# neeek2303/EMOPortraits

Measured on AMD Instinct MI355X. Metric: reenactment frames/sec @512x512, 1-src->N-driver, higher is better.
Workload: dtype f32

## Files before the change

### emoportraits_amd/build.py

```python
import concurrent.futures
import hashlib
import os
import subprocess
import sys

HERE = os.path.dirname(os.path.abspath(__file__))
CSRC = os.path.join(HERE, "csrc")
LIBDIR = os.path.join(HERE, "lib")
LIB = os.path.join(LIBDIR, "libemoportraits_hip.so")
OBJDIR = os.path.join(LIBDIR, "obj")
HIPCC = os.environ.get("HIPCC", "/opt/rocm/bin/hipcc")
ARCH = "gfx950"
FLAGS = ["--offload-arch=" + ARCH, "-O3", "-std=c++17", "-fPIC", "-ffp-contract=off", "-Wall",
         "-Wno-unused-function", "-Wno-unused-variable", "-mllvm", "-pragma-unroll-threshold=100000"]


EXTRA_FLAGS = {"gs3d_tile_pad_zeros.hip": ["-fno-slp-vectorize"], "gs3d_tile_pad_border.hip": ["-fno-slp-vectorize"],
               "gs3d_tile_pad_reflection.hip": ["-fno-slp-vectorize"],
               "conv_inst_bf16x3_3x3.hip": ["-fno-slp-vectorize"], "conv_inst_f16x2_3x3.hip": ["-fno-slp-vectorize"],
               "conv_inst_f16x2_ct2.hip": ["-fno-slp-vectorize"], "conv_inst_f16x2_p1.hip": ["-fno-slp-vectorize"],
               "conv_inst_f16x2_w8.hip": ["-fno-slp-vectorize"], "conv_inst_f16x2_up2.hip": ["-fno-slp-vectorize"]}


def sources():
    return sorted(os.path.join(CSRC, f) for f in os.listdir(CSRC) if f.endswith(".hip"))


def _digest(paths):
    h = hashlib.sha256()
    for p in sorted(paths):
        with open(p, "rb") as f:
            h.update(p.encode())
            h.update(f.read())
    h.update(" ".join(FLAGS).encode())
    for p in sorted(paths):
        h.update(" ".join(EXTRA_FLAGS.get(os.path.basename(p), [])).encode())
    return h.hexdigest()


def _compile(src):
    hdrs = [os.path.join(CSRC, f) for f in os.listdir(CSRC) if f.endswith(".h")]
    hdrs.append(os.path.join(HERE, "..", "include", "emo_hip.h"))
    dig = _digest([src] + hdrs)
    obj = os.path.join(OBJDIR, os.path.basename(src) + ".o")
    stamp = obj + ".sha"
    if os.path.exists(obj) and os.path.exists(stamp) and open(stamp).read() == dig:
        return obj, False
    extra = EXTRA_FLAGS.get(os.path.basename(src), [])
    cmd = [HIPCC] + FLAGS + extra + ["-c", src, "-o", obj]
    r = subprocess.run(cmd, capture_output=True, text=True)
    if r.returncode != 0:
        raise RuntimeError("hipcc failed for %s:\n%s\n%s" % (src, r.stdout, r.stderr))
    if r.stderr.strip():
        sys.stderr.write(r.stderr)
    with open(stamp, "w") as f:
        f.write(dig)
    return obj, True


def build_variant(name, defines):
    global FLAGS, OBJDIR, LIB
    saved = (FLAGS, OBJDIR, LIB)
    try:
        FLAGS = FLAGS + ["-D" + d for d in defines]
        OBJDIR = os.path.join(LIBDIR, "obj_" + name)
        LIB = os.path.join(LIBDIR, f"libemoportraits_hip_{name}.so")
        return build(force=False, verbose=True)
    finally:
        FLAGS, OBJDIR, LIB = saved


def build(force=False, verbose=True):
    os.makedirs(OBJDIR, exist_ok=True)
    srcs = sources()
    if force:
        for f in os.listdir(OBJDIR):
            os.remove(os.path.join(OBJDIR, f))
    with concurrent.futures.ThreadPoolExecutor(max_workers=min(8, len(srcs))) as ex:
        results = list(ex.map(_compile, srcs))
    objs = [o for o, _ in results]
    rebuilt = any(r for _, r in results)
    if rebuilt or not os.path.exists(LIB):
        cmd = [HIPCC, "--offload-arch=" + ARCH, "-shared", "-fPIC", "-o", LIB] + objs
        r = subprocess.run(cmd, capture_output=True, text=True)
        if r.returncode != 0:
            raise RuntimeError("link failed:\n%s\n%s" % (r.stdout, r.stderr))
        if verbose:
            print("built", LIB)
    elif verbose:
        print("up to date:", LIB)
    return LIB


if __name__ == "__main__":
    if "--variant" in sys.argv:
        i = sys.argv.index("--variant")
        build_variant(sys.argv[i + 1], sys.argv[i + 2:])
    else:
        build(force="--force" in sys.argv)
```

### emoportraits_amd/csrc/conv_api.hip

```cpp
#include "conv_dispatch.h"

conv_launch_fn conv_lookup_3x3_A(int, int);
conv_launch_fn conv_lookup_3x3_B(int, int);
conv_launch_fn conv_lookup_3x3_C(int, int);
conv_launch_fn conv_lookup_3x3_D(int, int);
conv_launch_fn conv_lookup_3x3_E(int, int);
conv_launch_fn conv_lookup_3x3_F(int, int);
conv_launch_fn conv_lookup_1x1_A(int, int);
conv_launch_fn conv_lookup_1x1_B(int, int);
conv_launch_fn conv_lookup_1x1_C(int, int);
conv_launch_fn conv_lookup_1x7_A(int, int);
conv_launch_fn conv_lookup_1x7_B(int, int);
conv_launch_fn conv_lookup_f16_3x3_D(int, int);
conv_launch_fn conv_lookup_f16_1x1_D(int, int);
conv_launch_fn conv_lookup_f16_3x3_G(int, int);
conv_launch_fn conv_lookup_bf16x3_3x3(int, int);
conv_launch_fn conv_lookup_f16x2_3x3(int, int);
conv_launch_fn conv_lookup_f16x2_1x1(int, int);
conv_launch_fn conv_lookup_f16x2_3x3_bm32(int, int);
conv_launch_fn conv_lookup_f16w8_3x3(int, int);
int conv_f16x2_up2_launch(ConvArgs, hipStream_t);

enum { PREC_F32 = 0, PREC_F16 = 1, PREC_S = 2, PREC_S2 = 3, PREC_H1 = 4, PREC_S2U = 5 };

static int shape_of_width(int Wl) {
  if (Wl >= 128 && Wl % 128 == 0) return SHAPE_W128;
  if (Wl == 64) return SHAPE_W64;
  if (Wl == 32) return SHAPE_W32;
  if (Wl == 16) return SHAPE_W16;
  if (Wl == 8) return SHAPE_W8;
  return -1;
}

static int kc_of(int KH, int KW, int cfg, int prec = PREC_F32) {
  if (prec == PREC_H1) return (cfg == CFG_D && KH == 3 && KW == 3) ? 32 : 0;
  if (prec == PREC_S2U) return (cfg == CFG_D && KH == 3 && KW == 3) ? 16 : 0;
  if (prec == PREC_S2 && cfg == CFG_D && KH == 1 && KW == 1) return 32;
  if (prec == PREC_S2 && cfg == CFG_F && KH == 3 && KW == 3) return 16;
  if (prec == PREC_S || prec == PREC_S2) return (cfg == CFG_D && KH == 3 && KW == 3) ? 16 : 0;
  if (prec == PREC_F16) {
    if (cfg == CFG_G) return (KH == 3 && KW == 3) ? EMO_CONV_KC_F16_3X3 : 0;
    if (cfg != CFG_D) return 0;
    return (KH == 3 && KW == 3) ? EMO_CONV_KC_F16_3X3 : (KH == 1 && KW == 1) ? EMO_CONV_KC_F16_1X1 : 0;
  }
  if (cfg == CFG_G) return 0;
  if (KH == 3 && KW == 3) return cfg == CFG_A ? EMO_CONV_KC_3X3_A : EMO_CONV_KC_3X3;
  if (cfg == CFG_D || cfg == CFG_E || cfg == CFG_F) return 0;
  if (KH == 1 && KW == 1) return EMO_CONV_KC_1X1;
  if (KH == 1 && KW == 7) return EMO_CONV_KC_1X7;
  return 0;
}

extern "C" int emo_conv_pack_info(int KH, int KW, int cfg, int* BM, int* KC) {
  if (!BM || !KC) return EMO_ERR_BAD_ARG;
  if (cfg == CFG_A) *BM = 128; else if (cfg == CFG_B || cfg == CFG_D || cfg == CFG_E) *BM = 64; else if (cfg == CFG_C || cfg == CFG_F) *BM = 32; else return EMO_ERR_BAD_ARG;
  *KC = kc_of(KH, KW, cfg);
  return *KC ? EMO_OK : EMO_ERR_UNSUPPORTED;
}

extern "C" int emo_conv_tile_positions(int cfg) {
  if (cfg == CFG_A || cfg == CFG_B || cfg == CFG_C) return 128;
  if (cfg == CFG_D || cfg == CFG_F || cfg == CFG_G) return 256;
  if (cfg == CFG_E) return 512;
  return EMO_ERR_BAD_ARG;
}

__global__ __launch_bounds__(256) void conv_splitk_epilogue_kernel(const float* __restrict__ partial,
                                                                   const float* __restrict__ bias, const float* res,
                                                                   float* out, long total, int ksplit, int Cout, int Dl,
                                                                   int Hl, int Wl, int act, int res_ups, const int* run_if) {
  if (run_if != nullptr && *run_if == 0) return;
  const long ovol = (long)Dl * Hl * Wl;
  for (long i = (long)blockIdx.x * 256 + threadIdx.x; i < total; i += (long)gridDim.x * 256) {
    float v = partial[i];
    for (int k = 1; k < ksplit; ++k) v += partial[(long)k * total + i];
    const long nc = i / ovol;
    if (bias) v += bias[nc % Cout];
    if (res) {
      if (res_ups) {
        const long sp = i - nc * ovol;
        const int x = (int)(sp % Wl);
        const long r = sp / Wl;
        const int y = (int)(r % Hl), z = (int)(r / Hl);
        const int Wr = Wl >> 1, Hr = Hl >> 1;
        v += res[nc * ((long)Dl * Hr * Wr) + ((long)z * Hr + (y >> 1)) * Wr + (x >> 1)];
      } else {
        v += res[i];
      }
    }
    out[i] = emo_act(v, act);
  }
}


extern "C" int emo_conv_pack_info_f16(int KH, int KW, int cfg, int* BM, int* KC) {
  if (!BM || !KC) return EMO_ERR_BAD_ARG;
  if (cfg == CFG_D) *BM = 64; else if (cfg == CFG_G) *BM = 128; else return EMO_ERR_UNSUPPORTED;
  *KC = kc_of(KH, KW, cfg, PREC_F16);
  return *KC ? EMO_OK : EMO_ERR_UNSUPPORTED;
}

extern "C" int emo_conv_pack_info_bf16x3(int KH, int KW, int cfg, int* BM, int* KC) {
  if (!BM || !KC) return EMO_ERR_BAD_ARG;
  if (cfg != CFG_D) return EMO_ERR_UNSUPPORTED;
  *BM = 64;
  *KC = kc_of(KH, KW, cfg, PREC_S);
  return *KC ? EMO_OK : EMO_ERR_UNSUPPORTED;
}

extern "C" int emo_conv_igemm_ksplit(int N, int Cin, int Cout, int D, int H, int W, int KD, int KH, int KW, int ups,
                                     int cfg) {
  const int kc = kc_of(KH, KW, cfg);
  if (!kc || N <= 0 || Cin <= 0 || Cout <= 0 || D <= 0 || H <= 0 || W <= 0 || cfg < 0 || cfg >= N_CFGS) return EMO_ERR_BAD_ARG;
  const int bm = (cfg == CFG_A || cfg == CFG_G) ? 128 : (cfg == CFG_B || cfg == CFG_D || cfg == CFG_E) ? 64 : 32;
  const int bp = (cfg == CFG_D || cfg == CFG_F || cfg == CFG_G) ? 256 : cfg == CFG_E ? 512 : 128;
  const long pos = (long)N * D * (ups ? 4 : 1) * H * W;
  const long blocks = ((pos + bp - 1) / bp) * ((Cout + bm - 1) / bm);
  const int nstages = ((Cin + kc - 1) / kc) * KD;
  long want = blocks >= 512 ? 1 : (512 + blocks - 1) / blocks;
  if (want > nstages / 8) want = nstages / 8;
  if (want > 16) want = 16;
  return want < 1 ? 1 : (int)want;
}

static int conv_igemm_dispatch(int prec, const float* x, const void* wpk, const float* bias, const float* scale,
                               const float* shift, const float* res, float* out, int N, int Cin, int Cout, int D, int H,
                               int W, int KD, int KH, int KW, int ups, int relu_in, int act, int res_ups, int cfg,
                               int ksplit, float* workspace, float* gn_stats, void* stream, float in_scale = 1.0f,
                               float w_scale = 1.0f, int* sat_flag = nullptr, const int* run_if = nullptr, int cot0 = 0,
                               int cot_end = 0) {
  if (!x || !wpk || !out) return EMO_ERR_BAD_ARG;
  if (gn_stats && ksplit > 1) return EMO_ERR_UNSUPPORTED;
  if ((long)D * H * W >= (1L << 30)) return EMO_ERR_UNSUPPORTED;
  if (ksplit < 1 || (ksplit > 1 && !workspace)) return EMO_ERR_BAD_ARG;
  if (N <= 0 || Cin <= 0 || Cout <= 0 || D <= 0 || H <= 0 || W <= 0) return EMO_ERR_BAD_ARG;
  if ((scale == nullptr) != (shift == nullptr)) return EMO_ERR_BAD_ARG;
  if (KD != 1 && KD != 3 && KD != 7) return EMO_ERR_UNSUPPORTED;
  if (KD == 3 && !(KH == 3 && KW == 3)) return EMO_ERR_UNSUPPORTED;
  if ((KD == 7) != (KH == 1 && KW == 7)) return EMO_ERR_UNSUPPORTED;
  if (cfg < 0 || cfg >= N_CFGS) return EMO_ERR_BAD_ARG;
  if (!emo_aligned16(wpk)) return EMO_ERR_ALIGN;
  if (ups && D != 1) return EMO_ERR_UNSUPPORTED;
  if ((long)Cin * D * H * W >= (1L << 31)) return EMO_ERR_UNSUPPORTED;
  ConvArgs a;
  a.x = x; a.wpk = reinterpret_cast<const float*>(wpk); a.bias = bias; a.scale = scale; a.shift = shift; a.res = res; a.out = out;
  a.N = N; a.Cin = Cin; a.Cout = Cout; a.D = D; a.H = H; a.W = W;
  a.Dl = D; a.Hl = ups ? 2 * H : H; a.Wl = ups ? 2 * W : W;
  a.KD = KD; a.relu_in = relu_in; a.act = act; a.res_ups = res_ups;
  a.gn_stats = gn_stats;
  a.n_cchunks = 0; a.tiles_x = a.tiles_y = a.tiles_z = 0; a.n_cotiles = 0; a.n_work = 0; a.cot0 = cot0; a.cot_end = cot_end;
  if ((cot0 != 0 && !(prec == PREC_F16 && cfg == CFG_D && ksplit == 1)) || (cot_end != 0 && prec != PREC_H1)) return EMO_ERR_BAD_ARG;
  a.in_scale = in_scale; a.out_scale = 1.0f / (in_scale * w_scale);
  a.sat_flag = sat_flag; a.run_if = run_if;
  const int shape = shape_of_width(a.Wl);
  if (shape < 0) return EMO_ERR_UNSUPPORTED;
  conv_launch_fn fn = nullptr;
  if (prec == PREC_H1) {
    if (!(KH == 3 && KW == 3 && (KD == 1 || KD == 3)) || cfg != CFG_D || Cin % 8 || ksplit != 1 || run_if != nullptr) return EMO_ERR_UNSUPPORTED;
    if (!(in_scale > 0.0f && w_scale > 0.0f)) return EMO_ERR_BAD_ARG;
    fn = conv_lookup_f16w8_3x3(a.Wl, ups);
  } else if (prec == PREC_S2U) {
    if (!(KH == 3 && KW == 3 && KD == 1) || !ups || cfg != CFG_D || ksplit != 1 || run_if != nullptr) return EMO_ERR_UNSUPPORTED;
    if (!(in_scale > 0.0f && w_scale > 0.0f)) return EMO_ERR_BAD_ARG;
    fn = &conv_f16x2_up2_launch;
  } else if (prec == PREC_S2 && KH == 1 && KW == 1) {
    if (KD != 1 || cfg != CFG_D || Cin % 8 || ksplit != 1 || run_if != nullptr) return EMO_ERR_UNSUPPORTED;
    if (!(in_scale > 0.0f && w_scale > 0.0f)) return EMO_ERR_BAD_ARG;
    fn = conv_lookup_f16x2_1x1(a.Wl, ups);
  } else if (prec == PREC_S2 && cfg == CFG_F) {
    if (!(KH == 3 && KW == 3 && (KD == 1 || KD == 3)) || Cin % 8) return EMO_ERR_UNSUPPORTED;
    if (!(in_scale > 0.0f && w_scale > 0.0f)) return EMO_ERR_BAD_ARG;
    fn = conv_lookup_f16x2_3x3_bm32(a.Wl, ups);
  } else if (prec == PREC_S || prec == PREC_S2) {
    if (!(KH == 3 && KW == 3 && (KD == 1 || KD == 3)) || cfg != CFG_D || Cin % 8) return EMO_ERR_UNSUPPORTED;
    if (prec == PREC_S2 && !(in_scale > 0.0f && w_scale > 0.0f)) return EMO_ERR_BAD_ARG;
    fn = prec == PREC_S ? conv_lookup_bf16x3_3x3(a.Wl, ups) : conv_lookup_f16x2_3x3(a.Wl, ups);
  } else if (prec == PREC_F16) {
    if (KD != 1 && !(KD == 3 && KH == 3)) return EMO_ERR_UNSUPPORTED;
    if ((cfg != CFG_D && cfg != CFG_G) || Cin % 8) return EMO_ERR_UNSUPPORTED;
    if (cfg == CFG_G) fn = (KH == 3 && KW == 3) ? conv_lookup_f16_3x3_G(shape, ups) : nullptr;
    else if (KH == 3 && KW == 3) fn = conv_lookup_f16_3x3_D(shape, ups);
    else if (KH == 1 && KW == 1) fn = conv_lookup_f16_1x1_D(shape, ups);
    else return EMO_ERR_UNSUPPORTED;
  } else if (cfg == CFG_G) {
    return EMO_ERR_UNSUPPORTED;
  } else if (cfg == CFG_D || cfg == CFG_E || cfg == CFG_F) {
    if (!(KH == 3 && KW == 3 && (KD == 1 || (KD == 3 && cfg != CFG_E)))) return EMO_ERR_UNSUPPORTED;
    fn = cfg == CFG_D ? conv_lookup_3x3_D(shape, ups) : cfg == CFG_E ? conv_lookup_3x3_E(shape, ups) : conv_lookup_3x3_F(shape, ups);
  } else if (KH == 3 && KW == 3) {
    fn = cfg == CFG_A ? conv_lookup_3x3_A(shape, ups) : cfg == CFG_B ? conv_lookup_3x3_B(shape, ups) : conv_lookup_3x3_C(shape, ups);
  } else if (KH == 1 && KW == 1) {
    fn = cfg == CFG_A ? conv_lookup_1x1_A(shape, ups) : cfg == CFG_B ? conv_lookup_1x1_B(shape, ups) : conv_lookup_1x1_C(shape, ups);
  } else if (KH == 1 && KW == 7) {
    fn = cfg == CFG_A ? conv_lookup_1x7_A(shape, ups) : cfg == CFG_B ? conv_lookup_1x7_B(shape, ups) : nullptr;
  } else {
    return EMO_ERR_UNSUPPORTED;
  }
  if (!fn) return EMO_ERR_UNSUPPORTED;
  const int kc = kc_of(KH, KW, cfg, prec);
  if (!kc) return EMO_ERR_UNSUPPORTED;
  const int nstages = ((Cin + kc - 1) / kc) * KD;
  if (ksplit > nstages) ksplit = nstages;
  a.stages_per_split = (nstages + ksplit - 1) / ksplit;
  a.ksplit = (nstages + a.stages_per_split - 1) / a.stages_per_split;
  a.partial = a.ksplit > 1 ? workspace : nullptr;
  const int rc = fn(a, (hipStream_t)stream);
  if (rc != EMO_OK || a.ksplit == 1) return rc;
  const long total = (long)N * Cout * a.Dl * a.Hl * a.Wl;
  long blocks = (total + 255) / 256;
  if (blocks > 262144) blocks = 262144;
  hipLaunchKernelGGL(conv_splitk_epilogue_kernel, dim3((unsigned)blocks), dim3(256), 0, (hipStream_t)stream, workspace, bias,
                     res, out, total, a.ksplit, Cout, a.Dl, a.Hl, a.Wl, act, res_ups, run_if);
  return emo_launch_status();
}

extern "C" int emo_conv_igemm_f32(const float* x, const float* wpk, const float* bias, const float* scale,
                                  const float* shift, const float* res, float* out, int N, int Cin, int Cout, int D,
                                  int H, int W, int KD, int KH, int KW, int ups, int relu_in, int act, int res_ups,
                                  int cfg, int ksplit, float* workspace, float* gn_stats, void* stream) {
  return conv_igemm_dispatch(PREC_F32, x, wpk, bias, scale, shift, res, out, N, Cin, Cout, D, H, W, KD, KH, KW, ups,
                             relu_in, act, res_ups, cfg, ksplit, workspace, gn_stats, stream);
}

extern "C" int emo_conv_igemm_f32_guarded(const float* x, const float* wpk, const float* bias, const float* scale,
                                          const float* shift, const float* res, float* out, int N, int Cin, int Cout, int D,
                                          int H, int W, int KD, int KH, int KW, int ups, int relu_in, int act, int res_ups,
                                          int cfg, int ksplit, float* workspace, float* gn_stats, void* stream,
                                          const int* run_if) {
  return conv_igemm_dispatch(PREC_F32, x, wpk, bias, scale, shift, res, out, N, Cin, Cout, D, H, W, KD, KH, KW, ups,
                             relu_in, act, res_ups, cfg, ksplit, workspace, gn_stats, stream, 1.0f, 1.0f, nullptr, run_if);
}

extern "C" int emo_conv_igemm_bf16x3(const float* x, const void* wpk3, const float* bias, const float* scale,
                                     const float* shift, const float* res, float* out, int N, int Cin, int Cout, int D,
                                     int H, int W, int KD, int KH, int KW, int ups, int relu_in, int act, int res_ups,
                                     int cfg, int ksplit, float* workspace, float* gn_stats, void* stream,
                                     const int* run_if) {
  return conv_igemm_dispatch(PREC_S, x, wpk3, bias, scale, shift, res, out, N, Cin, Cout, D, H, W, KD, KH, KW, ups,
                             relu_in, act, res_ups, cfg, ksplit, workspace, gn_stats, stream, 1.0f, 1.0f, nullptr, run_if);
}

extern "C" int emo_conv_igemm_f16x2(const float* x, const void* wpk2, const float* bias, const float* scale,
                                    const float* shift, const float* res, float* out, int N, int Cin, int Cout, int D,
                                    int H, int W, int KD, int KH, int KW, int ups, int relu_in, int act, int res_ups,
                                    int cfg, int ksplit, float* workspace, float* gn_stats, void* stream, float in_scale,
                                    float w_scale, int* overflow_flag) {
  if (cfg == EMO_CONV_CFG_F16X2_UP2)
    return conv_igemm_dispatch(PREC_S2U, x, wpk2, bias, scale, shift, res, out, N, Cin, Cout, D, H, W, KD, KH, KW, ups,
                               relu_in, act, res_ups, CFG_D, ksplit, workspace, gn_stats, stream, in_scale, w_scale,
                               overflow_flag, nullptr);
  return conv_igemm_dispatch(PREC_S2, x, wpk2, bias, scale, shift, res, out, N, Cin, Cout, D, H, W, KD, KH, KW, ups,
                             relu_in, act, res_ups, cfg, ksplit, workspace, gn_stats, stream, in_scale, w_scale,
                             overflow_flag, nullptr);
}

extern "C" int emo_conv_igemm_f16acc32(const float* x, const void* wpk16, const float* bias, const float* scale,
                                       const float* shift, const float* res, float* out, int N, int Cin, int Cout, int D,
                                       int H, int W, int KD, int KH, int KW, int ups, int relu_in, int act, int res_ups,
                                       int cfg, int ksplit, float* workspace, float* gn_stats, void* stream) {
  return conv_igemm_dispatch(PREC_F16, x, wpk16, bias, scale, shift, res, out, N, Cin, Cout, D, H, W, KD, KH, KW, ups,
                             relu_in, act, res_ups, cfg, ksplit, workspace, gn_stats, stream);
}

extern "C" int emo_conv_igemm_f16w8_rest(const float* x, const void* wpk1, const void* wpk16, const float* bias,
                                         const float* scale, const float* shift, const float* res, float* out, int N, int Cin,
                                         int Cout, int D, int H, int W, int KD, int KH, int KW, int ups, int relu_in, int act,
                                         int res_ups, int cfg, int ksplit, float* workspace, float* gn_stats, void* stream,
                                         float w_scale) {
  const int cot = (Cout + 63) / 64;
  if (!wpk16 || Cout % 64 || cot < 3 || !(cot & 1)) return EMO_ERR_UNSUPPORTED;
  const int Wl = ups ? 2 * W : W, Hl = ups ? 2 * H : H;
  if (!((Wl % 128 == 0 && Hl % 2 == 0) || (Wl == 64 && Hl % 4 == 0))) return EMO_ERR_UNSUPPORTED;
  int rc = conv_igemm_dispatch(PREC_H1, x, wpk1, bias, scale, shift, res, out, N, Cin, Cout, D, H, W, KD, KH, KW, ups, relu_in,
                               act, res_ups, cfg, ksplit, workspace, gn_stats, stream, 1.0f, w_scale, nullptr, nullptr, 0, cot - 1);
  if (rc != EMO_OK) return rc;
  return conv_igemm_dispatch(PREC_F16, x, wpk16, bias, scale, shift, res, out, N, Cin, Cout, D, H, W, KD, KH, KW, ups, relu_in,
                             act, res_ups, cfg, ksplit, workspace, gn_stats, stream, 1.0f, 1.0f, nullptr, nullptr, cot - 1, 0);
}

extern "C" int emo_conv_igemm_f16w8(const float* x, const void* wpk1, const float* bias, const float* scale,
                                    const float* shift, const float* res, float* out, int N, int Cin, int Cout, int D,
                                    int H, int W, int KD, int KH, int KW, int ups, int relu_in, int act, int res_ups,
                                    int cfg, int ksplit, float* workspace, float* gn_stats, void* stream, float w_scale) {
  return conv_igemm_dispatch(PREC_H1, x, wpk1, bias, scale, shift, res, out, N, Cin, Cout, D, H, W, KD, KH, KW, ups,
                             relu_in, act, res_ups, cfg, ksplit, workspace, gn_stats, stream, 1.0f, w_scale, nullptr, nullptr);
}
```

### emoportraits_amd/csrc/conv_igemm.h

```cpp
#pragma once
#include "common.h"

#include <mutex>
#include <set>
#include <utility>

typedef float floatx16 __attribute__((ext_vector_type(16)));
typedef float floatx4 __attribute__((ext_vector_type(4)));

#ifndef EMO_CONV_MAX_WAVES
#define EMO_CONV_MAX_WAVES 5
#endif

struct ConvArgs {
  const float* x;
  const float* wpk;
  const float* bias;
  const float* scale;
  const float* shift;
  const float* res;
  float* out;
  int N, Cin, Cout;
  int D, H, W;
  int Dl, Hl, Wl;
  int KD;
  int relu_in;
  int act;
  int res_ups;
  int n_cchunks;
  int tiles_x, tiles_y, tiles_z;
  int n_cotiles;
  int cot0;
  int cot_end;
  float in_scale, out_scale;
  int n_work;
  int ksplit;
  int stages_per_split;
  float* partial;
  float* gn_stats;
  int* sat_flag;
  const int* run_if;
};

template <int KH, int KW, int KC, int TZ, int TR, int TW, int TM, int TP, int WGM, int WGP, bool UPS>
struct ConvCfg {
  static constexpr int BM = WGM * TM * 32;
  static constexpr int BP = WGP * TP * 32;
  static constexpr int TAPS = KH * KW;
  static constexpr int KLOC = KC * TAPS;
  static constexpr int PR = TR + KH - 1;
  static constexpr int PW = TW + KW - 1;
  static constexpr int CHS = TZ * PR * PW;
  static constexpr int PATCH = KC * CHS;
  static constexpr int ASZ = KLOC * BM;
  static constexpr int BUF = ASZ + ((PATCH + 3) & ~3);
  static constexpr int SW = 4;
  static constexpr int THREADS = 256;
  static constexpr int WPC = KC >= SW ? 1 : SW / KC;
  static constexpr int CPW = KC >= SW ? KC / SW : 1;
  static constexpr int EPC = (CHS + 64 * WPC - 1) / (64 * WPC);
  static constexpr int NPE = CPW * EPC;
  static constexpr int NSTEPS = (KC / 2) * TAPS;
  static_assert(WGM * WGP == 4, "4 waves per block");
  static_assert(TZ * TR * TW == BP, "position tile must equal BP");
  static_assert(KC % 2 == 0 && (KC % SW == 0 || SW % KC == 0), "whole channels per wave, or whole waves per channel");
  static_assert(ASZ % 4 == 0, "weight tile must be float4-copyable");
  static_assert(TM * TP <= 8, "accumulator budget");
  static_assert(2 * BUF >= 2 * WGP * BM, "the GroupNorm tile statistics are exchanged through the stage buffers");
  static constexpr int LDS_BYTES = (2 * BUF + 256) * 4;
  static constexpr int BY_LDS = (160 * 1024) / LDS_BYTES;
  static constexpr int CAP = TM * TP >= 8 ? 2
                             : TM * TP >= 4 ? (EMO_CONV_MAX_WAVES < 4 ? EMO_CONV_MAX_WAVES : 4)
                                            : EMO_CONV_MAX_WAVES;
  static constexpr int OCC = BY_LDS < 2 ? 2 : (BY_LDS > CAP ? CAP : BY_LDS);
};

__device__ __forceinline__ float emo_act(float v, int act) {
  if (act == EMO_ACT_RELU) return fmaxf(v, 0.0f);
  if (act == EMO_ACT_TANH) return tanhf(v);
  if (act == EMO_ACT_SIGMOID) return 1.0f / (1.0f + expf(-v));
  return v;
}

#ifndef EMO_SGPR_HAZARD_NOP
#define EMO_SGPR_HAZARD_NOP "s_nop 4\n\t"
#endif


__device__ __forceinline__ float emo_gload_pinned(const float* sbase, unsigned voff) {
  float v;
  asm volatile(EMO_SGPR_HAZARD_NOP "global_load_dword %0, %1, %2" : "=v"(v) : "v"(voff), "s"(sbase) : "memory");
  return v;
}
__device__ __forceinline__ floatx4 emo_gload4_pinned(const float* sbase, unsigned voff) {
  floatx4 v;
  asm volatile(EMO_SGPR_HAZARD_NOP "global_load_dwordx4 %0, %1, %2" : "=v"(v) : "v"(voff), "s"(sbase) : "memory");
  return v;
}
__device__ __forceinline__ void emo_touch4(floatx4& v) { asm volatile("" : "+v"(v)); }
__device__ __forceinline__ void emo_wait_vmem0() { asm volatile("s_waitcnt vmcnt(0)" ::: "memory"); }
__device__ __forceinline__ void emo_touch(float& v) { asm volatile("" : "+v"(v)); }

#define acc_at(i_, j_) ((j_) < TPH ? acc_lo[i_][(j_) < TPH ? (j_) : 0] : acc_hi[i_][(j_) >= TPH ? (j_) - TPH : 0])

#ifndef EMO_CONV_NT_STORE
#define EMO_CONV_NT_STORE 0
#endif
__device__ __forceinline__ void emo_store4(float* p, const floatx4& v, bool aligned) {
  if (aligned) {
    if (EMO_CONV_NT_STORE) __builtin_nontemporal_store(v, reinterpret_cast<floatx4*>(p));
    else *reinterpret_cast<floatx4*>(p) = v;
  } else {
    p[0] = v[0]; p[1] = v[1]; p[2] = v[2]; p[3] = v[3];
  }
}

template <int TZ, int TR, int TW, int TM, int TP, int WGP, int BM>
__device__ __forceinline__ void conv_epilogue(const ConvArgs& a, floatx16 (&acc_lo)[TM][TP > 2 ? TP / 2 : TP],
                                              floatx16 (&acc_hi)[TM][TP > 2 ? TP / 2 : TP], float* smem, int n, int cotile,
                                              int ptile, int ks, int x0, int y0, int z0, int m0, int p0, int wp, int half,
                                              int l32, int tid) {
  constexpr int TPH = TP > 2 ? TP / 2 : TP;
  static_assert(TW % 4 == 0, "4 consecutive positions of a register quad lie in one tile row");
  const long plane = (long)a.Hl * a.Wl;
  const long ovol = (long)a.Dl * plane;
  const bool to_partial = a.partial != nullptr;
  const bool has_bias = a.bias != nullptr && !to_partial;
  const bool has_res = a.res != nullptr && !to_partial;
  const bool out_al = ((reinterpret_cast<unsigned long long>(to_partial ? a.partial : a.out) & 15ull) == 0);
  const bool res_al = has_res && ((reinterpret_cast<unsigned long long>(a.res) & 15ull) == 0);
#pragma unroll
  for (int i = 0; i < TM; ++i) {
    const int co = cotile * BM + m0 + i * 32 + l32;
    const bool co_ok = co < a.Cout;
    const int cs = co_ok ? co : a.Cout - 1;
    const float bv = has_bias ? a.bias[cs] : 0.0f;
#pragma unroll
    for (int j = 0; j < TP; ++j) {
      long sp[4];
      floatx4 rv[4];
#pragma unroll
      for (int q = 0; q < 4; ++q) {
        const int p4 = p0 + j * 32 + 8 * q + 4 * half;
        const int col = p4 % TW;
        const int row = (p4 / TW) % TR;
        const int pz = p4 / (TW * TR);
        const int z = z0 + pz, y = y0 + row, x = x0 + col;
        sp[q] = (long)z * plane + (long)y * a.Wl + x;
        rv[q] = floatx4{0.0f, 0.0f, 0.0f, 0.0f};
        if (has_res) {
          if (a.res_ups) {
            const int Wr = a.Wl >> 1, Hr = a.Hl >> 1;
            const float* rp = a.res + ((long)n * a.Cout + cs) * ((long)a.Dl * Hr * Wr) + ((long)z * Hr + (y >> 1)) * Wr + (x >> 1);
            const float r0 = rp[0], r1 = rp[1];
            rv[q] = floatx4{r0, r0, r1, r1};
          } else {
            const float* rp = a.res + ((long)n * a.Cout + cs) * ovol + sp[q];
            if (res_al) rv[q] = *reinterpret_cast<const floatx4*>(rp);
            else rv[q] = floatx4{rp[0], rp[1], rp[2], rp[3]};
          }
        }
      }
#pragma unroll
      for (int q = 0; q < 4; ++q) {
        floatx4 v;
        if (to_partial) {
#pragma unroll
          for (int e = 0; e < 4; ++e) v[e] = acc_at(i, j)[4 * q + e];
          if (co_ok) emo_store4(a.partial + (((long)ks * a.N + n) * a.Cout + co) * ovol + sp[q], v, out_al);
        } else {
#pragma unroll
          for (int e = 0; e < 4; ++e) {
            v[e] = emo_act(acc_at(i, j)[4 * q + e] + bv + rv[q][e], a.act);
            acc_at(i, j)[4 * q + e] = v[e];
          }
          if (co_ok) emo_store4(a.out + ((long)n * a.Cout + co) * ovol + sp[q], v, out_al);
        }
      }
    }
  }

  if (a.gn_stats != nullptr && !to_partial) {
    float* st_lds = smem;
    constexpr float inv_cnt = 1.0f / (float)(TP * 32);
#pragma unroll
    for (int i = 0; i < TM; ++i) {
      float s = 0.0f;
#pragma unroll
      for (int j = 0; j < TP; ++j)
#pragma unroll
        for (int r = 0; r < 16; ++r) s += acc_at(i, j)[r];
      s += __shfl_xor(s, 32);
      const float mean = s * inv_cnt;
      float m2 = 0.0f;
// ... 423 lines not shown
```

### emoportraits_amd/csrc/conv_inst_f16x2_3x3.hip

```cpp
#include "conv_dispatch.h"
#include "conv_igemm_bf16x3.h"
int conv_f16x2_ct2_4x64(ConvArgs, hipStream_t, int ups, int* rest_cot0);
int conv_f16x2_w8_4x64(ConvArgs, hipStream_t, int ups, int* rest_cot0);
template <bool UPS>
static int conv_f16x2_4x64(ConvArgs a, hipStream_t s) {
  int rest = 0;
  int rc = conv_f16x2_w8_4x64(a, s, UPS, &rest);
  if (rc != EMO_OK) return rc;
  if (rest == 0) rc = conv_f16x2_ct2_4x64(a, s, UPS, &rest);
  if (rc != EMO_OK) return rc;
  if (rest * ConvCfgS<4, 64, UPS, 2>::BM >= a.Cout) return EMO_OK;
  a.cot0 = rest;
  return conv_igemm_bf16x3_launch<4, 64, UPS, 2>(a, s);
}
conv_launch_fn conv_lookup_f16x2_3x3_bm32(int Wl, int ups) {
  if (Wl % 64 == 0 && !ups) return &conv_igemm_bf16x3_launch<4, 64, false, 2, 32>;
  return nullptr;
}
conv_launch_fn conv_lookup_f16x2_3x3(int Wl, int ups) {
  if (Wl % 64 == 0) return ups ? &conv_f16x2_4x64<true> : &conv_f16x2_4x64<false>;
  if (Wl == 32 && !ups) return &conv_igemm_bf16x3_launch<8, 32, false, 2>;
  if (Wl == 16 && !ups) return &conv_igemm_bf16x3_launch<16, 16, false, 2>;
  return nullptr;
}

#if EMO_S_TIMING
extern "C" int emo_debug_conv_timing_f16x2(unsigned long long* host_out, int n_items) {
  if (!host_out || n_items < 0 || n_items > EMO_S_TLOG_N) return EMO_ERR_BAD_ARG;
  if (hipDeviceSynchronize() != hipSuccess) return EMO_ERR_BAD_ARG;
  return hipMemcpyFromSymbol(host_out, HIP_SYMBOL(emo_s_tlog), (size_t)n_items * EMO_S_TLOG_W * sizeof(unsigned long long)) == hipSuccess ? EMO_OK : EMO_ERR_BAD_ARG;
}
#endif
```

Before: 411.3.

## Add z-streaming 3x3x3 f16x2 conv kernel reusing input planes across depth

Adds a new persistent kernel for the bm32 f16x2 3D 3x3x3 conv path that walks a run of consecutive depth slices. Each loaded input plane feeds all three kd taps into rotating accumulators, so input planes are loaded and converted once per slice instead of three times. It also overlaps the f16 conversion of the next chunk with the MFMA loop through sched_group_barriers. A heuristic picks the run length from the CU count, with a fallback to the old kernel when the shape does not fit. The cost is extra accumulator registers, one wave per EU, and halo slices recomputed at run boundaries.

```diff
diff --git a/emoportraits_amd/build.py b/emoportraits_amd/build.py
--- a/emoportraits_amd/build.py
+++ b/emoportraits_amd/build.py
@@ -19,7 +19,8 @@
                "gs3d_tile_pad_reflection.hip": ["-fno-slp-vectorize"],
                "conv_inst_bf16x3_3x3.hip": ["-fno-slp-vectorize"], "conv_inst_f16x2_3x3.hip": ["-fno-slp-vectorize"],
                "conv_inst_f16x2_ct2.hip": ["-fno-slp-vectorize"], "conv_inst_f16x2_p1.hip": ["-fno-slp-vectorize"],
-               "conv_inst_f16x2_w8.hip": ["-fno-slp-vectorize"], "conv_inst_f16x2_up2.hip": ["-fno-slp-vectorize"]}
+               "conv_inst_f16x2_w8.hip": ["-fno-slp-vectorize"], "conv_inst_f16x2_up2.hip": ["-fno-slp-vectorize"],
+               "conv_inst_f16x2_zs.hip": ["-fno-slp-vectorize"]}
 
 
 def sources():
diff --git a/emoportraits_amd/csrc/conv_api.hip b/emoportraits_amd/csrc/conv_api.hip
--- a/emoportraits_amd/csrc/conv_api.hip
+++ b/emoportraits_amd/csrc/conv_api.hip
@@ -151,7 +151,7 @@
   a.n_cchunks = 0; a.tiles_x = a.tiles_y = a.tiles_z = 0; a.n_cotiles = 0; a.n_work = 0; a.cot0 = cot0; a.cot_end = cot_end;
   if ((cot0 != 0 && !(prec == PREC_F16 && cfg == CFG_D && ksplit == 1)) || (cot_end != 0 && prec != PREC_H1)) return EMO_ERR_BAD_ARG;
   a.in_scale = in_scale; a.out_scale = 1.0f / (in_scale * w_scale);
-  a.sat_flag = sat_flag; a.run_if = run_if;
+  a.sat_flag = sat_flag; a.run_if = run_if; a.zrun = 0;
   const int shape = shape_of_width(a.Wl);
   if (shape < 0) return EMO_ERR_UNSUPPORTED;
   conv_launch_fn fn = nullptr;
diff --git a/emoportraits_amd/csrc/conv_igemm.h b/emoportraits_amd/csrc/conv_igemm.h
--- a/emoportraits_amd/csrc/conv_igemm.h
+++ b/emoportraits_amd/csrc/conv_igemm.h
@@ -40,6 +40,7 @@
   float* gn_stats;
   int* sat_flag;
   const int* run_if;
+  int zrun;
 };
 
 template <int KH, int KW, int KC, int TZ, int TR, int TW, int TM, int TP, int WGM, int WGP, bool UPS>
diff --git a/emoportraits_amd/csrc/conv_igemm_f16x2_zs.h b/emoportraits_amd/csrc/conv_igemm_f16x2_zs.h
--- /dev/null
+++ b/emoportraits_amd/csrc/conv_igemm_f16x2_zs.h
@@ -0,0 +1,325 @@
+#pragma once
+
+#ifndef EMO_Z_CONV_EARLY
+#define EMO_Z_CONV_EARLY 1
+#endif
+
+struct ConvCfgZ {
+  using S = ConvCfgS<4, 64, false, 2, 32>;
+  static constexpr int TR = 4, TW = 64, BM = 32, TP = 2, WGP = 4, KC = 16, NPL = 2;
+  static constexpr int WST = 3 * S::WROW;
+  static constexpr int WCH = 3 * WST;
+  static constexpr int NPIECE = WCH * 16 / 1024;
+  static constexpr int NDMA = (NPIECE + 3) / 4;
+  static constexpr int OFF_P = 0;
+  static constexpr int OFF_W = S::PBUF;
+  static constexpr int OFF_SCT = OFF_W + 2 * WCH;
+  static constexpr int SCT = 256;
+  static constexpr int OFF_BIAS_F = OFF_SCT * 4 + 2 * SCT;
+  static constexpr int OFF_STAT_F = OFF_BIAS_F + BM;
+  static constexpr int LDS_BYTES = (OFF_STAT_F + 2 * WGP * BM) * 4;
+  static constexpr int EPI_ROWF = S::EPI_ROWF, EPI_WAVE = S::EPI_WAVE;
+  static_assert(NPIECE * 1024 == WCH * 16 && NPIECE >= 4 * (NDMA - 1) + 2, "whole pieces; the last round holds >= 2");
+  static_assert(WGP * EPI_WAVE * 4 <= WCH * 16, "the epilogue transposes through the idle weight stage");
+  static_assert(LDS_BYTES <= 160 * 1024, "LDS");
+};
+
+template <int KD0, int KD1, typename F>
+__device__ __forceinline__ void conv_zs_mma(const char* lds_c, int w_off, const int (&b_off)[2][3],
+                                            floatx16 (&lo0)[1][2], floatx16 (&hi0)[1][2], floatx16 (&lo1)[1][2],
+                                            floatx16 (&hi1)[1][2], floatx16 (&lo2)[1][2], floatx16 (&hi2)[1][2], F&& convert) {
+  using Cfg = ConvCfgZ;
+  using S = Cfg::S;
+  constexpr int NK = KD1 - KD0 + 1;
+  constexpr int PA3[3] = {1, 0, 0}, PB3[3] = {0, 1, 0};
+  halfx8 fa[2][NK][2], fb[2][2][2];
+#define EMO_Z_FRAGS(set_, r_, s_)                                                                                     \
+  {                                                                                                                   \
+    _Pragma("unroll") for (int pl = 0; pl < 2; ++pl)                                                                  \
+      _Pragma("unroll") for (int j = 0; j < 2; ++j)                                                                   \
+        fb[set_][pl][j] = *reinterpret_cast<const halfx8*>(lds_c + b_off[j][s_] + ((r_) * S::NQ1 + Cfg::OFF_P + pl * S::PPL) * 16); \
+    _Pragma("unroll") for (int k = 0; k < NK; ++k)                                                                    \
+      _Pragma("unroll") for (int pl = 0; pl < 2; ++pl)                                                                \
+        fa[set_][k][pl] = *reinterpret_cast<const halfx8*>(lds_c + w_off + ((KD0 + k) * Cfg::WST + (r_) * S::WROW + pl * S::WPLANE + (s_) * 2 * Cfg::BM) * 16); \
+  }
+  EMO_Z_FRAGS(0, 0, 0)
+#pragma unroll
+  for (int gs = 0; gs < 9; ++gs) {
+    const int cur = gs & 1, nxt = cur ^ 1;
+    __builtin_amdgcn_sched_barrier(0);
+    if (gs < 8) EMO_Z_FRAGS(nxt, (gs + 1) / 3, (gs + 1) % 3)
+    if (EMO_Z_CONV_EARLY && gs >= 5) convert(gs - 5);
+#pragma unroll
+    for (int k = 0; k < NK; ++k)
+#pragma unroll
+      for (int p = 0; p < 3; ++p)
+#pragma unroll
+        for (int j = 0; j < 2; ++j) {
+          const int kd = KD0 + k;
+          const bool lead = PA3[p] == 0 && PB3[p] == 0;
+          floatx16& acc_ = kd == 0 ? (lead ? lo0[0][j] : hi0[0][j]) : kd == 1 ? (lead ? lo1[0][j] : hi1[0][j]) : (lead ? lo2[0][j] : hi2[0][j]);
+          acc_ = __builtin_amdgcn_mfma_f32_32x32x16_f16(fb[cur][PB3[p]][j], fa[cur][k][PA3[p]], acc_, 0, 0, 0);
+        }
+    if (EMO_Z_CONV_EARLY && gs >= 5) {
+#pragma unroll
+      for (int k = 0; k < 6 * NK; ++k) {
+        __builtin_amdgcn_sched_group_barrier(0x008, 1, 0);
+        if (gs < 8 && k < 4 + 2 * NK) __builtin_amdgcn_sched_group_barrier(0x100, (4 + 2 * NK + 6 * NK - 1) / (6 * NK), 0);
+        __builtin_amdgcn_sched_group_barrier(0x002, 3, 0);
+      }
+    } else if (gs < 8) {
+#pragma unroll
+      for (int k = 0; k < 4 + 2 * NK && k < 6 * NK; ++k) {
+        __builtin_amdgcn_sched_group_barrier(0x008, 1, 0);
+        __builtin_amdgcn_sched_group_barrier(0x100, (4 + 2 * NK + 6 * NK - 1) / (6 * NK), 0);
+      }
+    }
+    __builtin_amdgcn_sched_barrier(0);
+  }
+#undef EMO_Z_FRAGS
+}
+
+__device__ __forceinline__ void conv_f16x2_zs_body(const ConvArgs& a, float* smem, const unsigned smem_lds) {
+  using Cfg = ConvCfgZ;
+  using S = Cfg::S;
+  constexpr int BM = Cfg::BM, TP = Cfg::TP, WGP = Cfg::WGP, KC = Cfg::KC, TW = Cfg::TW, TR = Cfg::TR;
+  constexpr int PR = S::PR, NQ = S::NQ, NQ1 = S::NQ1, SUB = S::SUB, CHS = S::CHS, QPG = S::QPG, NHQ = S::NHQ, PPL = S::PPL;
+
+  const int tid = threadIdx.x;
+  const int lane = tid & 63;
+  const int wave = __builtin_amdgcn_readfirstlane(tid >> 6);
+  const int half = lane >> 5, l32 = lane & 31;
+  const int wp = wave;
+  float sat_m = 0.0f;
+
+  const int HW = a.H * a.W;
+  const long DHW = (long)a.D * HW;
+  const bool has_affine = a.scale != nullptr;
+  const int epi_mode = __builtin_amdgcn_readfirstlane(
+      (a.act != EMO_ACT_NONE || a.Cout % BM != 0 || (long)a.Dl * a.Hl * a.Wl > (1l << 23) ||
+       (reinterpret_cast<unsigned long long>(a.out) & 15ull) != 0) ? -1
+      : a.res == nullptr ? 0
+      : (!a.res_ups && (reinterpret_cast<unsigned long long>(a.res) & 15ull) == 0) ? 1 : -1);
+  constexpr float CLAMP_HI = 65504.0f;
+  const float clamp_lo = a.relu_in ? 0.0f : -CLAMP_HI;
+  const int ncc = a.n_cchunks;
+  const int nruns = (a.D + a.zrun - 1) / a.zrun;
+
+  const int q_u = tid % QPG;
+  const int q_g = __builtin_amdgcn_readfirstlane(tid / QPG);
+  const bool is_quad = q_u < PR * NQ;
+  const int hq = q_u - PR * NQ;
+  const bool is_halo = !is_quad && hq < NHQ;
+  const int h_side = hq & 1;
+  const int q_r = is_quad ? q_u / NQ : (is_halo ? hq >> 1 : 0);
+  const int q_c = is_quad ? q_u - q_r * NQ : 0;
+  int q_slb[4];
+#pragma unroll
+  for (int i = 0; i < 4; ++i) {
+    const int dump = q_g * CHS + i * SUB + PR * NQ1 + (q_u & 3);
+    const int own = is_quad ? q_g * CHS + i * SUB + q_r * NQ1 + q_c : q_g * CHS + h_side * SUB + q_r * NQ1 + NQ;
+    q_slb[i] = ((is_quad || (is_halo && i == (h_side ? 0 : 3))) ? own : dump) * 16;
+  }
+  const int a_off = (half * BM + l32) * 16;
+  int b_off[2][3];
+#pragma unroll
+  for (int j = 0; j < 2; ++j) {
+    const int p = wp * TP * 32 + j * 32 + l32;
+    const int col = p % TW, row = p / TW;
+#pragma unroll
+    for (int s = 0; s < 3; ++s) {
+      const int pc = col + s - 1;
+      const int slot = pc < 0 ? row * NQ1 + NQ : (pc >= TW ? SUB + row * NQ1 + NQ : (pc & 3) * SUB + row * NQ1 + (pc >> 2));
+      b_off[j][s] = (half * CHS + slot) * 16;
+    }
+  }
+  const char* const lds_c = reinterpret_cast<const char*>(smem);
+  char* const lds_w = reinterpret_cast<char*>(smem);
+  float* const sct = smem + Cfg::OFF_SCT * 4;
+  const unsigned lane16 = (unsigned)lane * 16u;
+  unsigned usoff[8];
+#pragma unroll
+  for (int u = 0; u < 8; ++u) usoff[u] = (unsigned)__builtin_amdgcn_readfirstlane((int)((unsigned)u * (unsigned)DHW * 4u));
+
+  floatx4 qv[8];
+  halfx8 cv_h[4], cv_m[4];
+  floatx4 q_sc[2], q_sh[2];
+  float q_lo = 0.0f, q_hi = 0.0f;
+  int q_tix = 0;
+  floatx16 acc_lo[3][1][2], acc_hi[3][1][2];
+
+  for (int L = blockIdx.x; L < a.n_work; L += gridDim.x) {
+    int rest = L;
+    const int cot_ = rest % a.n_cotiles; rest /= a.n_cotiles;
+    const int run_ = rest % nruns; rest /= nruns;
+    const int tx_ = rest % a.tiles_x; rest /= a.tiles_x;
+    const int ty_ = rest % a.tiles_y; rest /= a.tiles_y;
+    const int it_cotile = __builtin_amdgcn_readfirstlane(cot_);
+    const int it_n = __builtin_amdgcn_readfirstlane(rest);
+    const int it_x0 = __builtin_amdgcn_readfirstlane(tx_ * TW), it_y0 = __builtin_amdgcn_readfirstlane(ty_ * TR);
+    const int ptile_yx = __builtin_amdgcn_readfirstlane(ty_ * a.tiles_x + tx_);
+    const int zb = __builtin_amdgcn_readfirstlane(run_ * a.zrun);
+    const int nout = min(a.zrun, a.D - zb);
+    const int zi_last = min(zb + nout, a.D - 1);
+    const int zi_first = zb > 0 ? zb - 1 : 0;
+
+    const int q_y = it_y0 - 1 + q_r;
+    const int q_x = is_quad ? it_x0 + 4 * q_c : (h_side ? it_x0 + TW : it_x0 - 4);
+    const bool lq_ok = (is_quad || is_halo) && (unsigned)q_y < (unsigned)a.H && q_x >= 0 && q_x < a.W;
+    const unsigned lq_off = lq_ok ? (unsigned)(q_y * a.W + q_x) * 4u : 0u;
+    const emo_intx4 xrs = emo_raw_buffer(a.x + (long)it_n * a.Cin * DHW);
+    const char* const wsrc = reinterpret_cast<const char*>(a.wpk) + (long)it_cotile * ncc * (Cfg::WCH * 16);
+
+#define EMO_Z_ISSUE(zi_, cc_, wb_)                                                                                    \
+  {                                                                                                                   \
+    const char* const wp_ = wsrc + (long)(cc_) * (Cfg::WCH * 16);                                                     \
+    _Pragma("unroll") for (int k = 0; k < Cfg::NDMA; ++k) {                                                           \
+      const int j = k < Cfg::NDMA - 1 ? wave + 4 * k : 4 * (Cfg::NDMA - 1) + (wave & 1);                              \
+      emo_dma16_pinned_s(wp_ + j * 1024, lane16, smem_lds + (unsigned)((Cfg::OFF_W + (wb_) * Cfg::WCH) * 16 + j * 1024)); \
+    }                                                                                                                 \
+    const int c0_ = (cc_) * KC + q_g * 8;                                                                             \
+    const bool cv_ = c0_ < a.Cin;                                                                                     \
+    const int cs_ = cv_ ? c0_ : 0;                                                                                    \
+    const bool keep_ = lq_ok && cv_;                                                                                  \
+    q_lo = keep_ ? clamp_lo : 0.0f;                                                                                   \
+    q_hi = keep_ ? CLAMP_HI : 0.0f;                                                                                   \
+    q_tix = cs_ >> 2;                                                                                                 \
+    const unsigned q_vo = lq_off + ((unsigned)cs_ * (unsigned)DHW + (unsigned)((zi_) * HW)) * 4u;                     \
+    _Pragma("unroll") for (int u = 0; u < 8; u += 2) emo_bload4x2_pinned(xrs, q_vo, usoff[u], usoff[u + 1], qv[u], qv[u + 1]); \
+  }
+#define EMO_Z_CONVERT_PX(i_)                                                                                          \
+  {                                                                                                                   \
+    if ((i_) == 0) {                             \
+      const floatx4* t4_ = reinterpret_cast<const floatx4*>(sct) + q_tix;                                             \
+      q_sc[0] = t4_[0]; q_sc[1] = t4_[1]; q_sh[0] = t4_[Cfg::SCT / 4]; q_sh[1] = t4_[Cfg::SCT / 4 + 1];               \
+    }                                                                                                                 \
+    _Pragma("unroll") for (int hf = 0; hf < 2; ++hf) {                                                                \
+      float t_[4];                                                                                                    \
+      _Pragma("unroll") for (int k = 0; k < 4; ++k) t_[k] = __fmaf_rn(qv[4 * hf + k][i_], q_sc[hf][k], q_sh[hf][k]);  \
+      sat_m = __builtin_fmaxf(__builtin_fmaxf(sat_m, __builtin_fabsf(t_[0])), __builtin_fabsf(t_[1]));                \
+      sat_m = __builtin_fmaxf(__builtin_fmaxf(sat_m, __builtin_fabsf(t_[2])), __builtin_fabsf(t_[3]));                \
+      _Pragma("unroll") for (int k = 0; k < 4; k += 2)                                                                \
+        emo_split_f16x2_pair(__builtin_amdgcn_fmed3f(t_[k], q_lo, q_hi), __builtin_amdgcn_fmed3f(t_[k + 1], q_lo, q_hi), \
+                             cv_h[i_], cv_m[i_], 4 * hf + k);                                                         \
+    }                                                                                                                 \
+  }
+#define EMO_Z_STORE_PATCH()                                                                                           \
+  {                                                                                                                   \
+    _Pragma("unroll") for (int i = 0; i < 4; ++i) {                                                                   \
+      char* d_ = lds_w + q_slb[i] + Cfg::OFF_P * 16;                                                                  \
+      *reinterpret_cast<halfx8*>(d_) = cv_h[i];                                                                       \
+      *reinterpret_cast<halfx8*>(d_ + PPL * 16) = cv_m[i];                                                            \
+    }                                                                                                                 \
+  }
+#define EMO_Z_LANDED() { emo_wait_vmem0(); _Pragma("unroll") for (int u = 0; u < 8; ++u) emo_touch4(qv[u]); }
+
+    {
+      float te_sc = 1.0f, te_sh = 0.0f, te_b = 0.0f;
+      if (has_affine && tid < a.Cin) {
+        te_sc = a.scale[(long)it_n * a.Cin + tid];
+        te_sh = a.shift[(long)it_n * a.Cin + tid];
+      }
+      if (tid < BM && a.bias != nullptr) {
+        const int co_ = it_cotile * BM + tid;
+        te_b = a.bias[co_ < a.Cout ? co_ : a.Cout - 1];
+      }
+      if (tid < Cfg::SCT) {
+        sct[tid] = te_sc * a.in_scale;
+        sct[Cfg::SCT + tid] = te_sh * a.in_scale;
+      }
+      if (tid < BM) smem[Cfg::OFF_BIAS_F + (tid >> 5) * 32 + (tid & 3) * 8 + ((tid & 31) >> 2)] = te_b;
+    }
+    __syncthreads();
+    EMO_Z_ISSUE(zi_first, 0, 0)
+#pragma unroll
+    for (int st = 0; st < 3; ++st)
+#pragma unroll
+      for (int j = 0; j < 2; ++j)
+#pragma unroll
+        for (int r = 0; r < 16; ++r) { acc_lo[st][0][j][r] = 0.0f; acc_hi[st][0][j][r] = 0.0f; }
+    EMO_Z_LANDED()
+#pragma unroll
+    for (int i = 0; i < 4; ++i) EMO_Z_CONVERT_PX(i)
+    EMO_Z_STORE_PATCH()
+    __syncthreads();
+
+    int wb = 0;
+#define EMO_Z_EPI_FAST(RES_, lo_, hi_)                                                                                \
+  {                                                                                                                   \
+    floatx4 rv_[8];                                                                                                   \
+    conv_epilogue_fast_issue<TW, TP, BM, RES_, 0>(a, rv_, it_n, it_cotile, it_x0, it_y0, zo_, wp, lane);              \
+    conv_epilogue_fast_finish<TW, 1, TP, WGP, BM, 2, Cfg::EPI_ROWF, RES_>(a, lo_, hi_, rv_, scratch_, smem + Cfg::OFF_BIAS_F, \
+                                                                          smem + Cfg::OFF_STAT_F, it_n, it_cotile, ptile_, it_x0, \
+                                                                          it_y0, zo_, wp, half, l32, lane, tid);      \
+  }
+    for (int t = 0; t < nout + 2; ++t) {
+      const int zi_ = zb - 1 + t;
+      if ((unsigned)zi_ < (unsigned)a.D) {
+        for (int cc = 0; cc < ncc; ++cc) {
+          const bool last_cc_ = cc + 1 == ncc;
+          const int nzi_ = last_cc_ ? zi_ + 1 : zi_, ncc_ = last_cc_ ? 0 : cc + 1;
+          const bool has_next_ = nzi_ <= zi_last;
+          EMO_Z_ISSUE(has_next_ ? nzi_ : zi_, has_next_ ? ncc_ : cc, wb ^ 1)
+          auto convert_ = [&](int i) __attribute__((always_inline)) {
+            if (i == 0) EMO_Z_LANDED()
+            EMO_Z_CONVERT_PX(i)
+          };
+          conv_zs_mma<0, 2>(lds_c, a_off + (Cfg::OFF_W + wb * Cfg::WCH) * 16, b_off, acc_lo[0], acc_hi[0], acc_lo[1], acc_hi[1],
+                            acc_lo[2], acc_hi[2], convert_);
+          if (!EMO_Z_CONV_EARLY) {
+#pragma unroll
+            for (int i = 0; i < 4; ++i) convert_(i);
+          }
+          __syncthreads();
+          EMO_Z_STORE_PATCH()
+          __syncthreads();
+          wb ^= 1;
+        }
+      }
+      if (t >= 2) {
+        const int zo_ = zb + t - 2;
+        const int ptile_ = zo_ * (a.tiles_x * a.tiles_y) + ptile_yx;
+        float* const scratch_ = smem + (Cfg::OFF_W + (wb ^ 1) * Cfg::WCH) * 4 + wave * Cfg::EPI_WAVE;
+        if (epi_mode == 1) EMO_Z_EPI_FAST(1, acc_lo[2], acc_hi[2])
+        else if (epi_mode == 0) EMO_Z_EPI_FAST(0, acc_lo[2], acc_hi[2])
+        else {
+          conv_epilogue_rows<TR, TW, 1, TP, WGP, BM, 2, Cfg::EPI_ROWF>(a, acc_lo[2], acc_hi[2], scratch_, smem + Cfg::OFF_BIAS_F,
+                                                                       smem + Cfg::OFF_STAT_F, it_n, it_cotile, ptile_, 0, it_x0,
+                                                                       it_y0, zo_, wp, half, l32, lane, tid);
+#if defined(__HIP_DEVICE_COMPILE__)
+          __builtin_amdgcn_s_waitcnt(0x0F70);
+#endif
+        }
+        __syncthreads();
+      }
+#pragma unroll
+      for (int j = 0; j < 2; ++j) {
+        acc_lo[2][0][j] = acc_lo[1][0][j]; acc_hi[2][0][j] = acc_hi[1][0][j];
+        acc_lo[1][0][j] = acc_lo[0][0][j]; acc_hi[1][0][j] = acc_hi[0][0][j];
+#pragma unroll
+        for (int r = 0; r < 16; ++r) { acc_lo[0][0][j][r] = 0.0f; acc_hi[0][0][j][r] = 0.0f; }
+      }
+    }
+#undef EMO_Z_EPI_FAST
+#undef EMO_Z_LANDED
+#undef EMO_Z_STORE_PATCH
+#undef EMO_Z_CONVERT_PX
+#undef EMO_Z_ISSUE
+  }
+  if (a.sat_flag != nullptr && sat_m > 65504.0f) *a.sat_flag = 1;
+}
+
+static inline int conv_f16x2_zs_run_length(int N, int Cout, int D, int H, int W, int ncu) {
+  constexpr int RMIN = 6;
+  if (D < RMIN || H % ConvCfgZ::TR || W % ConvCfgZ::TW || ncu < 1) return 0;
+  const long base = (long)N * (H / ConvCfgZ::TR) * (W / ConvCfgZ::TW) * ((Cout + ConvCfgZ::BM - 1) / ConvCfgZ::BM);
+  if (base * ((D + RMIN - 1) / RMIN) < ncu) return 0;
+  int best = 0;
+  long best_cost = 0;
+  for (int r = RMIN; r <= D; ++r) {
+    const long items = base * ((D + r - 1) / r);
+    const long cost = ((items + ncu - 1) / ncu) * (r + 2);
+    if (best == 0 || cost <= best_cost) { best = r; best_cost = cost; }
+  }
+  return best;
+}
diff --git a/emoportraits_amd/csrc/conv_inst_f16x2_3x3.hip b/emoportraits_amd/csrc/conv_inst_f16x2_3x3.hip
--- a/emoportraits_amd/csrc/conv_inst_f16x2_3x3.hip
+++ b/emoportraits_amd/csrc/conv_inst_f16x2_3x3.hip
@@ -2,6 +2,7 @@
 #include "conv_igemm_bf16x3.h"
 int conv_f16x2_ct2_4x64(ConvArgs, hipStream_t, int ups, int* rest_cot0);
 int conv_f16x2_w8_4x64(ConvArgs, hipStream_t, int ups, int* rest_cot0);
+int conv_f16x2_bm32_4x64(ConvArgs, hipStream_t);
 template <bool UPS>
 static int conv_f16x2_4x64(ConvArgs a, hipStream_t s) {
   int rest = 0;
@@ -14,7 +15,7 @@
   return conv_igemm_bf16x3_launch<4, 64, UPS, 2>(a, s);
 }
 conv_launch_fn conv_lookup_f16x2_3x3_bm32(int Wl, int ups) {
-  if (Wl % 64 == 0 && !ups) return &conv_igemm_bf16x3_launch<4, 64, false, 2, 32>;
+  if (Wl % 64 == 0 && !ups) return &conv_f16x2_bm32_4x64;
   return nullptr;
 }
 conv_launch_fn conv_lookup_f16x2_3x3(int Wl, int ups) {
diff --git a/emoportraits_amd/csrc/conv_inst_f16x2_zs.hip b/emoportraits_amd/csrc/conv_inst_f16x2_zs.hip
--- /dev/null
+++ b/emoportraits_amd/csrc/conv_inst_f16x2_zs.hip
@@ -0,0 +1,57 @@
+#include "conv_dispatch.h"
+#include "conv_igemm_bf16x3.h"
+#include "conv_igemm_f16x2_zs.h"
+
+__global__ __launch_bounds__(256) __attribute__((amdgpu_waves_per_eu(1, 1)))
+void conv_igemm_f16x2_zs_kernel(const ConvArgs a) {
+  extern __shared__ __attribute__((aligned(16))) float smem[];
+  const unsigned smem_lds = (unsigned)(size_t)(__attribute__((address_space(3))) char*)reinterpret_cast<char*>(smem);
+  conv_f16x2_zs_body(a, smem, smem_lds);
+}
+
+static int conv_f16x2_zs_choose(int N, int Cout, int D, int H, int W, int ncu) {
+  const char* e = getenv("EMO_CONV_ZS_RUN");
+  if (e && *e) {
+    const int k = atoi(e);
+    if (k <= 0 || H % ConvCfgZ::TR || W % ConvCfgZ::TW) return 0;
+    return k < D ? k : D;
+  }
+  return conv_f16x2_zs_run_length(N, Cout, D, H, W, ncu);
+}
+
+static int zs_last_run = 0;
+
+int conv_f16x2_bm32_4x64(ConvArgs a, hipStream_t s) {
+  zs_last_run = 0;
+  const bool fits = a.KD == 3 && a.ksplit == 1 && a.run_if == nullptr && a.cot0 == 0 && !a.res_ups && a.Cin % 8 == 0 &&
+                    a.Cin <= ConvCfgZ::SCT && a.D == a.Dl && a.H == a.Hl && a.W == a.Wl && a.N <= 65535 &&
+                    (unsigned long long)a.Cin * a.D * a.H * a.W * 4ull < (1ull << 32) &&
+                    (reinterpret_cast<unsigned long long>(a.x) & 15ull) == 0;
+  const int ncu = emo_cu_count();
+  const int run = fits ? conv_f16x2_zs_choose(a.N, a.Cout, a.D, a.H, a.W, ncu) : 0;
+  if (run <= 0) return conv_igemm_bf16x3_launch<4, 64, false, 2, 32>(a, s);
+  a.tiles_x = a.Wl / ConvCfgZ::TW;
+  a.tiles_y = a.Hl / ConvCfgZ::TR;
+  a.tiles_z = a.Dl;
+  a.n_cchunks = (a.Cin + ConvCfgZ::KC - 1) / ConvCfgZ::KC;
+  a.n_cotiles = (a.Cout + ConvCfgZ::BM - 1) / ConvCfgZ::BM;
+  a.stages_per_split = a.n_cchunks * a.KD;
+  a.partial = nullptr;
+  a.zrun = run;
+  const long items = (long)a.N * a.tiles_y * a.tiles_x * ((a.D + run - 1) / run) * a.n_cotiles;
+  if (items > 0x7fffffffL || (long)a.tiles_x * a.tiles_y * a.tiles_z > 0x7fffffffL) return EMO_ERR_UNSUPPORTED;
+  a.n_work = (int)items;
+  auto kern = conv_igemm_f16x2_zs_kernel;
+  const int rc = emo_raise_dynamic_lds(kern);
+  if (rc != EMO_OK) return rc;
+  const int grid = a.n_work > ncu ? ncu : a.n_work;
+  hipLaunchKernelGGL(kern, dim3((unsigned)grid), dim3(256), (size_t)ConvCfgZ::LDS_BYTES, s, a);
+  zs_last_run = run;
+  return emo_launch_status();
+}
+
+extern "C" int emo_debug_conv_zs_run(int N, int Cout, int D, int H, int W, int ncu) {
+  if (ncu <= 0) return conv_f16x2_zs_choose(N, Cout, D, H, W, emo_cu_count());
+  return conv_f16x2_zs_run_length(N, Cout, D, H, W, ncu);
+}
+extern "C" int emo_debug_conv_zs_last_run(void) { return zs_last_run; }
```

Result: faster. 415.6, median of 6 (+1.0%).
